# shahruk10/kaldi-tflite

Measured on AMD Instinct MI355X. Metric: x-vectors/sec (10 s @16 kHz), higher is better.
Workload: dtype f16mx

## Files before the change

### include/ktf_hip.h

```cpp
#ifndef KTF_HIP_H_
#define KTF_HIP_H_

#include <stddef.h>
#include <stdint.h>

#ifdef __cplusplus
extern "C" {
#endif

#define KTF_OK 0
#define KTF_EINVAL (-1)
#define KTF_ELAUNCH (-2)
#define KTF_EUNSUPPORTED (-3)

#define KTF_F32 0
#define KTF_BF16 1
#define KTF_BF16P 3

#define KTF_GEMM_F32 0
#define KTF_GEMM_BF16 1
#define KTF_GEMM_BF16X3 2
#define KTF_GEMM_F16MX 5
#define KTF_GEMM_BF16X4 6

// ... 51 lines not shown
    int32_t mel_stride;
    int32_t reserved;
} KtfFrontendTables;

#define KTF_IN_WAV 0
#define KTF_IN_FRAMES 1
#define KTF_IN_WINDOWED 2
#define KTF_IN_WAV_I16 3
#define KTF_OUT_FRAMES 0
#define KTF_OUT_WINDOWED 1
#define KTF_OUT_FBANK 2
#define KTF_OUT_MFCC 3

int64_t ktf_num_frames(int64_t n_samples, int32_t frame_size, int32_t frame_shift);
int64_t ktf_num_frames_padded(int64_t n_samples, int32_t frame_size, int32_t frame_shift, int32_t pad_mode);

int ktf_frontend_f32(const void* in, int64_t B, int64_t n, int32_t in_kind, const KtfFrontendCfg* cfg,
                     const KtfFrontendTables* tab, int32_t out_stage, float* out, float* energy,
                     uint64_t seed, void* stream);

int ktf_dct_f32(const float* x, int64_t rows, int32_t in_dim, int32_t out_dim, const float* dct,
                const float* lifter, float* out, void* stream);

typedef struct KtfVadCfg {
    float energy_threshold;
    float energy_mean_scale;
    float proportion_threshold;
    int32_t frames_context;
    int32_t energy_coeff;
} KtfVadCfg;

typedef struct KtfCmvnCfg {
    int32_t window;
    int32_t norm_vars;
    int32_t valid;
    int32_t reserved;
} KtfCmvnCfg;

int ktf_vad_mask_f32(const float* feats, int64_t B, int64_t T, int32_t D, const KtfVadCfg* cfg, float* mask,
                     void* stream);
int ktf_vad_index(const float* feats, int64_t B, int64_t T, int32_t D, const KtfVadCfg* cfg, int32_t* idx,
                  int32_t* lens, void* stream);
int ktf_cmvn_f32(const float* x, int64_t B, int64_t T, int32_t D, int64_t ldx, const int32_t* lens,
                 const KtfCmvnCfg* cfg, float* out, int64_t ldo, int32_t* out_lens, float* work, void* stream);
int ktf_vad_cmvn(const float* feats, int64_t B, int64_t T, int32_t D, const KtfVadCfg* vad, const KtfCmvnCfg* cmvn,
                 void* out, int32_t out_dtype, int64_t ldo, int32_t* lens, int32_t* idx_work, float* work,
                 void* stream);

typedef struct KtfVcPlan {
    int64_t pos_ints;
    int64_t stage_floats;
    int64_t bs_floats;
    int64_t col_floats;
    int64_t lds_bytes;
    int32_t nsplit;
    int32_t lds_form;
} KtfVcPlan;
int ktf_vad_cmvn_plan(int64_t B, int64_t T, int32_t D, int64_t ldo, KtfVcPlan* plan);
int ktf_cmvn_plan(int64_t T, int32_t D, int64_t ldo, KtfVcPlan* plan);

int ktf_route_short(const int32_t* lens, int64_t B, int32_t min_frames, int32_t* lens_main, int32_t* lens_short, int32_t* host_flag,
                    int32_t seq, void* stream);

typedef struct KtfTdnnDesc {
    int32_t units;
    int32_t din;
    int32_t din_pad;
    int32_t nctx;
    int32_t ctx[16];
    int32_t subsampling;
    int32_t valid;
    int32_t act;
    int32_t gemm;
    int32_t x_dtype, w_dtype, y_dtype;
    int32_t flags;
} KtfTdnnDesc;

#define KTF_TDNN_REF_TILES 1
#define KTF_TDNN_DET_STATS 2
#define KTF_TDNN_K_INTERLEAVED 4
#define KTF_TDNN_W_TILED 8

#define KTF_TDNN_MX_LOADER (1 << 24)

const char* ktf_tdnn_last_kernel(void);


int64_t ktf_tdnn_out_len(int64_t len, const KtfTdnnDesc* d);
int ktf_tdnn_out_lens(const int32_t* lens, int64_t B, const KtfTdnnDesc* d, int32_t* out_lens, void* stream);

int ktf_tdnn(const void* x, int64_t B, int64_t T, int64_t ldx, const int32_t* lens, const KtfTdnnDesc* d,
             const void* w, const void* w_lo, const float* bias, const float* scale, const float* shift,
             void* y, int64_t ldy, int32_t* out_lens, void* stream);

int ktf_tdnn_stats(const void* x, int64_t B, int64_t T, int64_t ldx, const int32_t* lens, const KtfTdnnDesc* d,
                   const void* w, const void* w_lo, const float* bias, const float* scale, const float* shift, double* sums,
                   void* stream);
int ktf_tdnn_split(const void* x_hi, const void* x_lo, int64_t B, int64_t T, int64_t ldx, const int32_t* lens,
                   const KtfTdnnDesc* d, const void* w, const void* w_lo, const float* bias, const float* scale,
                   const float* shift, void* y, void* y_lo, int64_t ldy, int32_t* out_lens, void* stream);
int ktf_tdnn_split_flat(const void* x_hi, const void* x_lo, int64_t B, int64_t T, int64_t ldx, const int32_t* row_starts, const int32_t* row_map,
                        const KtfTdnnDesc* d, const void* w, const void* w_lo, const float* bias, const float* scale,
                        const float* shift, void* y, void* y_lo, int64_t ldy, void* stream);
int64_t ktf_flat_stats_slots(int64_t T);
int64_t ktf_flat_row_map_rows(int64_t B, int64_t T);
int ktf_flat_row_map(const int32_t* row_starts, int64_t B, int64_t T, int32_t* map, void* stream);
int ktf_tdnn_split_flat_stats(const void* x_hi, const void* x_lo, int64_t B, int64_t T, int64_t ldx, const int32_t* row_starts,
                              const int32_t* row_map, const KtfTdnnDesc* d, const void* w, const void* w_lo, const float* bias, const float* scale,
                              const float* shift, double* sums, void* stream);
int ktf_stats_finalize_flat(const double* sums, int64_t slots, const int32_t* row_starts, int64_t T, int64_t B, int32_t D,
                            int32_t include_std, float eps, float* out, int64_t ld_out, void* stream);
int ktf_tdnn_split_stats(const void* x_hi, const void* x_lo, int64_t B, int64_t T, int64_t ldx, const int32_t* lens,
                         const KtfTdnnDesc* d, const void* w, const void* w_lo, const float* bias, const float* scale,
                         const float* shift, double* sums, void* stream);
int ktf_split_bf16(const float* src, int64_t rows, int32_t D, int64_t ld_src, void* hi, void* lo, int64_t ld_dst,
                   void* stream);
int ktf_split_bf16_rows(const float* src, int64_t B, int64_t T, int32_t D, int64_t ld_src, const int32_t* lens, void* hi, void* lo,
                        int64_t ld_dst, void* stream);
int ktf_mx_planes(const float* src, int64_t B, int64_t T, int32_t D, int64_t ld_src, const int32_t* lens, void* xh, void* xl4,
                  void* x4, void* xs, void* stream);
int ktf_tdnn_mx(const void* xh, const void* xl4, const void* x4, const void* xs, int64_t B, int64_t T, const int32_t* lens,
                const KtfTdnnDesc* d, const void* wh, const void* wq, const float* bias, const float* scale, const float* shift,
                void* yh, void* yl4, void* y4, void* ys, float* yf, int64_t ldy, void* stream);
int ktf_tdnn_mx_flat(const void* xh, const void* xl4, const void* x4, const void* xs, int64_t B, int64_t T, const int32_t* row_starts,
                     const int32_t* row_map, const KtfTdnnDesc* d, const void* wh, const void* wq, const float* bias, const float* scale,
                     const float* shift, void* yh, void* yl4, void* y4, void* ys, void* stream);
int ktf_tdnn_mx_flat_stats(const void* xh, const void* xl4, const void* x4, const void* xs, int64_t B, int64_t T, const int32_t* row_starts,
                           const int32_t* row_map, const KtfTdnnDesc* d, const void* wh, const void* wq, const float* bias, const float* scale,
                           const float* shift, double* sums, void* stream);
int ktf_tdnn_mx_stats(const void* xh, const void* xl4, const void* x4, const void* xs, int64_t B, int64_t T, const int32_t* lens,
                      const KtfTdnnDesc* d, const void* wh, const void* wq, const float* bias, const float* scale,
                      const float* shift, double* sums, void* stream);
int ktf_stats_finalize(const double* sums, const int32_t* lens, int64_t T, int64_t B, int32_t D, int32_t include_std,
                       float eps, float* out, int64_t ld_out, void* stream);
int64_t ktf_stats_slots(int64_t T);
int64_t ktf_tdnn_stats_slots(int64_t T, int32_t gemm);
int32_t ktf_tdnn_slot_rows(int32_t gemm);
int64_t ktf_mx_stats_slots(int64_t T, int32_t flags);
int32_t ktf_mx_slot_rows(int32_t flags);
int ktf_stats_finalize_slots(const double* sums, int64_t slots, int32_t slot_rows, const int32_t* lens, int64_t T, int64_t B, int32_t D,
                             int32_t include_std, float eps, float* out, int64_t ld_out, void* stream);

int ktf_activation_f32(float* y, int64_t B, int64_t T, int32_t D, int64_t ld, const int32_t* lens, int32_t act, const float* scale,
                       const float* shift, void* stream);

int ktf_affine_act_f32(const float* x, int64_t rows, int32_t D, int32_t act, const float* scale, const float* shift,
                       float* y, void* stream);
int ktf_convert_pad(const void* src, int32_t src_dtype, int64_t rows, int32_t D, int64_t ld_src, void* dst,
                    int32_t dst_dtype, int64_t ld_dst, void* stream);

int ktf_stats_pool(const void* x, int32_t x_dtype, int64_t B, int64_t T, int32_t D, int64_t ldx,
                   const int32_t* lens, int32_t input_period, int32_t include_std, float eps, float* out,
                   int64_t ld_out, void* stream);
int ktf_stats_pool_windowed_f32(const float* x, int64_t B, int64_t T, int32_t D, int32_t left, int32_t right,
                                int32_t input_period, int32_t output_period, int32_t start, int64_t T_out,
                                int32_t include_std, float eps, float* out, void* stream);

int ktf_xvec_tail_f32(const float* pooled, int64_t ld_pooled, const double* sums, int64_t slots, int32_t slot_rows, const int32_t* lens, int64_t T,
                      int64_t B, int32_t D, int32_t include_std, float eps, const float* W, int64_t ldw, const float* bias,
                      int32_t units, const float* mean, const float* A, const float* off, int32_t out_dim, float* partial,
                      uint32_t* counters, float* y, float* h_out, int32_t group, int32_t flags, void* stream);
#define KTF_TAIL_SKIP_EMPTY 1
int ktf_xvec_post_f32(const float* x, int64_t B, int32_t in_dim, int32_t out_dim, const float* mean, const float* A,
                      const float* off, float* y, void* stream);

int ktf_plda_f64(const double* x, int64_t B, int32_t dim, const double* A, const double* offset, const double* psi,
// ... 180 lines not shown
```

### kaldi-tflite_amd/csrc/tdnn_mx.hip

```cpp
#include "tdnn_mx_common.h"

#define MXP_ROWS 256
__global__ __launch_bounds__(MXP_ROWS) void mx_planes_kernel(const float* __restrict__ src, int64_t T, int64_t ld, int D,
                                                             const int32_t* __restrict__ lens, char* __restrict__ xh,
                                                             char* __restrict__ xl4, char* __restrict__ x4, char* __restrict__ xs) {
    __shared__ float tile[MXP_ROWS * 33];
    const int b = blockIdx.z, c = blockIdx.y, nch = gridDim.y;
    const int64_t t0 = (int64_t)blockIdx.x * MXP_ROWS;
    const int64_t len = lens ? (int64_t)lens[b] : T;
    if (t0 >= len) return;
    const int rows = (int)(len - t0 < MXP_ROWS ? len - t0 : MXP_ROWS);
    const int tid = threadIdx.x;
    const float* base = src + ((int64_t)b * T + t0) * ld + c * 32;
    const bool vec = (ld & 3) == 0 && ((uintptr_t)src & 15) == 0 && c * 32 + 32 <= ld;
#pragma unroll
    for (int k = 0; k < 8; ++k) {
        const int q = k * MXP_ROWS + tid, r = q >> 3, e4 = (q & 7) * 4;
        if (r < rows) {
            float v[4];
            if (vec) {
                const f32x4 t = *reinterpret_cast<const f32x4*>(base + (int64_t)r * ld + e4);
                const int nd = D - (c * 32 + e4);
                v[0] = nd > 0 ? t.x : 0.0f; v[1] = nd > 1 ? t.y : 0.0f; v[2] = nd > 2 ? t.z : 0.0f; v[3] = nd > 3 ? t.w : 0.0f;
            } else {
// ... 127 lines not shown
        }
        s_row = er[2].y;
        s_lm1 = er[2].z - 1;
        s_ub = er[2].x < 0 ? 0u : (unsigned)(er[2].x - er[2].y) * (unsigned)p.nch_in;
    }
    const unsigned vw = (unsigned)tid * 16u;
    const int wave_k0 = (int)(unsigned)(size_t)(lds_ptr_t*)(rsm + wave * 1024);
    [[maybe_unused]] const int wave_k = wave_k0;
#define MX_LDS_AT(off_, c_) ((lds_ptr_t*)(size_t)(unsigned)((off_) + (c_)))
    int kb[5], ko[5];
    kb[0] = MX_KQ_BIAS;
    ko[0] = MX_CTX(0);
#define MX_DMA_A_E(ks_, e_, n_)                                                                                        \
    {                                                                                                                  \
        int r_ = a_row[n_] + ko[e_];                                                                                   \
        const int hi_ = FLAT ? a_lm1[n_] : lenm1;                                                                      \
        r_ = r_ < 0 ? 0 : (r_ > hi_ ? hi_ : r_);                                                                       \
        const unsigned vo_ = ((FLAT ? a_ub[n_] : 0u) + (unsigned)r_) * 64u + a_cb[n_];                                 \
        __builtin_amdgcn_raw_ptr_buffer_load_lds(r_xh, MX_LDS_AT(wave_k, ((ks_) & 1) * MX_STAGE + (n_) * 8192), 16, vo_, kb[e_] << 6, 0, 0); \
    }
#define MX_DMA_A_I(ks_, e_, n_)                                                                                        \
    __builtin_amdgcn_raw_ptr_buffer_load_lds(r_xh, MX_LDS_AT(wave_k, ((ks_) & 1) * MX_STAGE + (n_) * 8192), 16, (n_) ? va1 : va0, \
                                             (kb[e_] + ko[e_]) << 6, 0, 0);
#define MX_DMA_A(ks_, e_, n_) { if constexpr (INTERIOR) MX_DMA_A_I(ks_, e_, n_) else MX_DMA_A_E(ks_, e_, n_) }
#define MX_DMA_W(ks_, n_)                                                                                              \
    __builtin_amdgcn_raw_ptr_buffer_load_lds(r_wh, MX_LDS_AT(wave_k, ((ks_) & 1) * MX_STAGE + MX_TILE + (n_) * 8192), 16, vw, \
                                             (ks_) * MX_TILE + (n_) * 8192, 0, 0);
    MX_DMA_W(0, 0) MX_DMA_W(0, 1) MX_DMA_A_E(0, 0, 0) MX_DMA_A_E(0, 0, 1)
    const __amdgpu_buffer_rsrc_t r_xl4 = mx_rsrc_pinned(p.xl4 + (ub - MX_KQ_BIAS) * 16);
    const __amdgpu_buffer_rsrc_t r_x4 = mx_rsrc_pinned(p.x4 + (ub - MX_KQ_BIAS) * 16);
    const __amdgpu_buffer_rsrc_t r_xs = mx_rsrc_pinned(p.xs + (ub - MX_KQ_BIAS) * 4);
    if constexpr (FLAT) {
        if (p.nctx == 1 && MX_CTX(0) == 0) {
            interior = true;
        } else if (out_len == 256) {
            const i32x4 e0 = flat_row(0), e1 = flat_row(255);
            interior = __builtin_amdgcn_readfirstlane(e0.w) == __builtin_amdgcn_readfirstlane(e1.w) &&
                       __builtin_amdgcn_readfirstlane(e0.y) + MX_CTX(0) >= 0 &&
                       __builtin_amdgcn_readfirstlane(e1.y) + MX_CTX(p.nctx - 1) <= __builtin_amdgcn_readfirstlane(e1.z) - 1;
        }
    }
    [[maybe_unused]] const unsigned va0 = (a_ub[0] + (unsigned)a_row[0]) * 64u + a_cb[0], va1 = (a_ub[1] + (unsigned)a_row[1]) * 64u + a_cb[1];
    [[maybe_unused]] const unsigned vs16 = (s_ub + (unsigned)s_row) * 16u, vs4 = (s_ub + (unsigned)s_row) * 4u;

    const int sa_k0 = (int)(unsigned)(size_t)(lds_ptr_t*)(rsm + (wave & 3) * 1024 + (wave >> 2) * 4096);
    const int sa_ks0 = (int)(unsigned)(size_t)(lds_ptr_t*)(rsm + (wave & 3) * 256 + (wave >> 2) * 1024);
    const bool wave_hi = wave >= 4;

    int* const tkb = reinterpret_cast<int*>(rsm + MX_KQ_OFF);
    int* const tko = tkb + (nkp + 4);

#define MX_DMA_SA(n_)                                                                                                  \
    {                                                                                                                  \
        constexpr int plane_ = ((n_) < 4 ? (n_) : 0) >> 1, h_ = (n_) < 4 ? ((n_) & 1) : (n_) - 4;                      \
        unsigned rec_ = 0u;                                                                                            \
        int so_;                                                                                                       \
        if constexpr (INTERIOR) {                                                                                      \
            so_ = sk_b[h_] + sk_o[h_];                                                                                 \
        } else {                                                                                                       \
            int r_ = s_row + sk_o[h_];                                                                                 \
            const int hi_ = FLAT ? s_lm1 : lenm1;                                                                      \
            r_ = r_ < 0 ? 0 : (r_ > hi_ ? hi_ : r_);                                                                   \
            rec_ = (FLAT ? s_ub : 0u) + (unsigned)r_;                                                                  \
            so_ = sk_b[h_];                                                                                            \
        }                                                                                                              \
        if ((n_) < 4) {                                                                                                \
            __builtin_amdgcn_raw_ptr_buffer_load_lds(plane_ ? r_x4 : r_xl4, MX_LDS_AT(sa_k, MX_SA_OFF + plane_ * 16384 + h_ * 8192), 16, \
                                                     INTERIOR ? vs16 : rec_ * 16u, so_ << 4, 0, 0);                    \
        } else {                                                                                                       \
            __builtin_amdgcn_raw_ptr_buffer_load_lds(r_xs, MX_LDS_AT(sa_ks, MX_SA_OFF + 32768 + h_ * 2048), 4, INTERIOR ? vs4 : rec_ * 4u, so_ << 2, 0, 0); \
        }                                                                                                              \
    }
#define MX_DMA_SW(ss_, n_)                                                                                             \
    __builtin_amdgcn_raw_ptr_buffer_load_lds(r_wq, MX_LDS_AT(wave_k, MX_SW_OFF + (n_) * 8192), 16, vw, (ss_) * MX_WQ_BLOCK + (n_) * 8192, 0, 0);

    f32x4 acc[8][4];
    const int r16 = lane & 15, q4 = lane >> 4;
    const int fr = (4 - ((r16 >> 2) & 3)) & 3;
    const int coff = ((q4 ^ fr) << 4);
    const int a_row_off = (wm * 128 + r16) * 64 + coff;
    const int b_row_off = (wn * 64 + r16) * 64 + coff;
    const int klim = PADK ? p.nk : nkp;

    auto kloop = [&](auto itag) {
        constexpr bool INTERIOR = decltype(itag)::value;
        {
            unsigned char* const prm_w = rsm + MX_PRM_OFF + (wave & 3) * 256;
            const unsigned vcol = (unsigned)(n0 + (wave & 3) * 64 + lane) * 4u;
            const float* const vec0 = wave_hi ? p.scale : p.bias;
            if (vec0) __builtin_amdgcn_raw_ptr_buffer_load_lds(mx_rsrc(vec0, p.units * 4), (lds_ptr_t*)(prm_w + (wave_hi ? 1024 : 0)), 4, vcol, 0, 0, 0);
            else reinterpret_cast<float*>(prm_w + (wave_hi ? 1024 : 0))[lane] = wave_hi ? 1.0f : 0.0f;
            if (!wave_hi) {
                if (p.shift) __builtin_amdgcn_raw_ptr_buffer_load_lds(mx_rsrc(p.shift, p.units * 4), (lds_ptr_t*)(prm_w + 2048), 4, vcol, 0, 0, 0);
                else reinterpret_cast<float*>(prm_w + 2048)[lane] = 0.0f;
            }
        }
        for (int k = tid; k < nkp + 4; k += 512) {
            const int kk = k + 1 < p.nk ? k + 1 : 0;
            const int ch = kk / p.nctx, ci = kk - ch * p.nctx;
            tkb[k] = ch * (int)p.T + MX_KQ_BIAS;
            tko[k] = MX_CTX(ci);
        }
        {
            int ch = 0, ci = 0;
#pragma unroll
            for (int e = 1; e <= 4; ++e) {
                if (++ci == p.nctx) { ci = 0; ++ch; }
                const bool real = e < p.nk;
                kb[e] = (real ? ch * (int)p.T : 0) + MX_KQ_BIAS;
                ko[e] = real ? MX_CTX(ci) : MX_CTX(0);
            }
        }
#pragma unroll
        for (int i = 0; i < 8; ++i)
#pragma unroll
            for (int j = 0; j < 4; ++j) acc[i][j] = f32x4{0.0f, 0.0f, 0.0f, 0.0f};
        for (int ss = 0; ss < p.nss; ++ss) {
            i32x4 tb_n, to_n;
            int sk_b[2], sk_o[2];
            int wave_k = wave_k0, sa_k = sa_k0, sa_ks = sa_ks0;
            asm volatile("" : "+s"(wave_k), "+s"(sa_k), "+s"(sa_ks));
#pragma unroll
            for (int j = 0; j < 4; ++j) {
                const int ks = 4 * ss + j;
                if (j == 1 || j == 2) asm volatile("s_waitcnt vmcnt(6)" ::: "memory");
                else if (j == 0) asm volatile("s_waitcnt vmcnt(0) lgkmcnt(0)" ::: "memory");
                else asm volatile("s_waitcnt vmcnt(0)" ::: "memory");
                __builtin_amdgcn_s_barrier();
                asm volatile("" ::: "memory");
                const bool live = PADK ? ks < p.nk : true;
#define MX_NEXT() ({ int k1_ = ks + 1; asm volatile("" : "+s"(k1_)); k1_ < klim; })
                const unsigned char* sa = rsm + (ks & 1) * MX_STAGE;
                const unsigned char* sw = sa + MX_TILE;
                hfrag8 bh[4];
                hfrag8 a_cur, a_nx1;
                if (live) {
#pragma unroll
                    for (int jj = 0; jj < 4; ++jj) bh[jj] = *reinterpret_cast<const hfrag8*>(sw + b_row_off + jj * 1024);
                    a_cur = *reinterpret_cast<const hfrag8*>(sa + a_row_off);
                    a_nx1 = *reinterpret_cast<const hfrag8*>(sa + a_row_off + 1024);
                }
                __builtin_amdgcn_sched_barrier(0);
                if (MX_NEXT()) { MX_DMA_A(ks + 1, j + 1, 0) MX_DMA_A(ks + 1, j + 1, 1) }
                __builtin_amdgcn_sched_barrier(0);
#pragma unroll
                for (int i = 0; i < 8; ++i) {
                    if (live) {
                        acc[i][0] = __builtin_amdgcn_mfma_f32_16x16x32_f16(a_cur, bh[0], acc[i][0], 0, 0, 0);
                        __builtin_amdgcn_sched_barrier(0);
                        hfrag8 a_nx2 = a_nx1;
                        if (i < 6) a_nx2 = *reinterpret_cast<const hfrag8*>(sa + a_row_off + (i + 2) * 1024);
#pragma unroll
                        for (int jj = 1; jj < 4; ++jj) acc[i][jj] = __builtin_amdgcn_mfma_f32_16x16x32_f16(a_cur, bh[jj], acc[i][jj], 0, 0, 0);
                        a_cur = a_nx1;
                        a_nx1 = a_nx2;
                    }
                    __builtin_amdgcn_sched_barrier(0);
                    if (i == 0) { if (MX_NEXT()) MX_DMA_W(ks + 1, 0) }
                    if (i == 1) { if (MX_NEXT()) MX_DMA_W(ks + 1, 1) }
                    if (j == 0) {
                        if (i == 1) {
                            sk_b[0] = wave_hi ? kb[1] : kb[0]; sk_o[0] = wave_hi ? ko[1] : ko[0];
                            sk_b[1] = wave_hi ? kb[3] : kb[2]; sk_o[1] = wave_hi ? ko[3] : ko[2];
                        }
                        if (i == 2) MX_DMA_SA(0)
                        if (i == 3) MX_DMA_SA(1)
                        if (i == 4) MX_DMA_SA(2)
                        if (i == 5) MX_DMA_SA(3)
                        if (i == 6) MX_DMA_SA(4)
                        if (i == 7) MX_DMA_SA(5)
                    }
                    if (j == 1) {
                        if (i == 2) MX_DMA_SW(ss, 0)
                        if (i == 3) MX_DMA_SW(ss, 1)
                        if (i == 4) MX_DMA_SW(ss, 2)
                        if (i == 5) MX_DMA_SW(ss, 3)
                        if (i == 6) MX_DMA_SW(ss, 4)
                        if (i == 7) MX_DMA_SW(ss, 5)
                    }
                    if (j == 2 && i == 3) {
                        tb_n = *reinterpret_cast<const i32x4*>(tkb + 4 * ss + 4);
                        to_n = *reinterpret_cast<const i32x4*>(tko + 4 * ss + 4);
                    }
                    __builtin_amdgcn_sched_barrier(0);
                }
#undef MX_NEXT
            }
            __builtin_amdgcn_sched_barrier(0);
            {
                int tl;
                asm volatile("v_mbcnt_lo_u32_b32 %0, -1, 0\n\tv_mbcnt_hi_u32_b32 %0, -1, %0" : "=v"(tl));
                const int sw_rec = ((tl & 63) >> 4) * 256 + wn * 64 + (tl & 15);
                const int sa_rec = ((tl & 63) >> 4) * 256 + wm * 128 + (tl & 15);
                unsigned o_a16 = MX_SA_OFF + sa_rec * 16, o_a4 = MX_SA_OFF + 32768 + sa_rec * 4;
                asm volatile("" : "+v"(o_a16), "+v"(o_a4));
                const unsigned char* const pa16 = rsm + o_a16;
                const unsigned char* const pa4 = rsm + o_a4;
                unsigned o_w16 = MX_SW_OFF + sw_rec * 16, o_w8 = MX_SW_OFF + 32768 + sw_rec * 8, o_w4 = MX_SW_OFF + 40960 + sw_rec * 4;
                asm volatile("" : "+v"(o_w16), "+v"(o_w8), "+v"(o_w4));
                const unsigned char* const pw16 = rsm + o_w16;
                const unsigned char* const pw8 = rsm + o_w8;
                const unsigned char* const pw4 = rsm + o_w4;
                u32x4 w4[4], wl6a[4];
                u32x2 wl6b[4];
                unsigned wsc[4];
#pragma unroll
                for (int jj = 0; jj < 4; ++jj) {
                    w4[jj] = *reinterpret_cast<const u32x4*>(pw16 + jj * 256);
                    wl6a[jj] = *reinterpret_cast<const u32x4*>(pw16 + 16384 + jj * 256);
                    wl6b[jj] = *reinterpret_cast<const u32x2*>(pw8 + jj * 128);
                    wsc[jj] = *reinterpret_cast<const unsigned*>(pw4 + jj * 64);
                }
                u32x4 l_n = *reinterpret_cast<const u32x4*>(pa16);
                u32x4 h_n = *reinterpret_cast<const u32x4*>(pa16 + 16384);
                unsigned s_n = *reinterpret_cast<const unsigned*>(pa4);
#pragma unroll
                for (int i = 0; i < 8; ++i) {
                    const u32x4 l = l_n, h = h_n;
                    const unsigned asc = s_n;
                    if (i < 7) {
                        l_n = *reinterpret_cast<const u32x4*>(pa16 + (i + 1) * 256);
                        h_n = *reinterpret_cast<const u32x4*>(pa16 + 16384 + (i + 1) * 256);
                        s_n = *reinterpret_cast<const unsigned*>(pa4 + (i + 1) * 64);
                    }
                    const i32x8 al = i32x8{(int)l.x, (int)l.y, (int)l.z, (int)l.w, 0, 0, 0, 0};
                    const i32x8 ah = i32x8{(int)h.x, (int)h.y, (int)h.z, (int)h.w, 0, 0, 0, 0};
#pragma unroll
                    for (int jj = 0; jj < 4; ++jj) {
                        const i32x8 bw = i32x8{(int)w4[jj].x, (int)w4[jj].y, (int)w4[jj].z, (int)w4[jj].w, 0, 0, 0, 0};
                        acc[i][jj] = __builtin_amdgcn_mfma_scale_f32_16x16x128_f8f6f4(al, bw, acc[i][jj], 4, 4, 0, asc, 0, wsc[jj]);
                    }
#pragma unroll
                    for (int jj = 0; jj < 4; ++jj) {
                        const i32x8 bw = i32x8{(int)wl6a[jj].x, (int)wl6a[jj].y, (int)wl6a[jj].z, (int)wl6a[jj].w, (int)wl6b[jj].x, (int)wl6b[jj].y, 0, 0};
                        acc[i][jj] = __builtin_amdgcn_mfma_scale_f32_16x16x128_f8f6f4(ah, bw, acc[i][jj], 4, 2, 1, asc, 1, wsc[jj]);
                    }
                    if (i == 3) {
                        kb[0] = kb[4];
                        ko[0] = ko[4];
#pragma unroll
                        for (int e = 0; e < 4; ++e) {
                            kb[e + 1] = __builtin_amdgcn_readfirstlane(tb_n[e]);
                            ko[e + 1] = __builtin_amdgcn_readfirstlane(to_n[e]);
                        }
                    }
                    __builtin_amdgcn_sched_barrier(0);
                }
            }
        }
    };
    if constexpr (FLAT) {
        if (interior) kloop(std::true_type{});
        else kloop(std::false_type{});
    } else {
        kloop(std::false_type{});
    }
#undef MX_DMA_A
#undef MX_DMA_A_E
#undef MX_DMA_A_I
#undef MX_DMA_W
#undef MX_DMA_SA
#undef MX_DMA_SW
#undef MX_ARG_BATCH
#undef MX_LDS_AT
#undef MX_CTX

#include "tdnn_mx_epilogue.inc"
}

template <int ACT, int OUT, bool PADK, bool FLAT = false>
__global__ __launch_bounds__(512) void tdnn_mx_kernel(MxParams p, int mtiles, int ntiles, int gtiles, double* __restrict__ stats) {
    extern __shared__ __attribute__((aligned(16))) unsigned char rsm[];
    mx_tile<ACT, OUT, PADK, FLAT>(p, blockIdx.x, mtiles, ntiles, gtiles, stats, rsm);
}

static int mx_launch(const void* xh, const void* xl4, const void* x4, const void* xs, int64_t B, int64_t T, const int32_t* lens,
                     const KtfTdnnDesc* d, const void* wh, const void* wq, const float* bias, const float* scale, const float* shift,
                     void* yh, void* yl4, void* y4, void* ys, float* yf, int64_t ldy, double* stats, void* stream, const char* who,
                     const int32_t* row_starts = nullptr, const int32_t* row_map = nullptr) {
    KTF_REQUIRE(d && wh && wq, "%s: null argument", who);
    KTF_REQUIRE(d->gemm == KTF_GEMM_F16MX, "%s: needs KTF_GEMM_F16MX", who);
    KTF_REQUIRE(B >= 0 && T >= 0 && B < 65536, "%s: bad size", who);
    KTF_REQUIRE(B == 0 || T == 0 || (xh && xl4 && x4 && xs), "%s: null argument", who);
    if (const int rc = tdnn_check_desc(d, scale, shift, who); rc != KTF_OK) return rc;
    KTF_REQUIRE(d->subsampling <= 64, "%s: subsampling %d outside [1,64]", who, d->subsampling);
    const bool plain = !d->valid && d->subsampling == 1;
    KTF_REQUIRE(plain || !stats, "%s: the fused pooling takes SAME padding without subsampling", who);
    KTF_REQUIRE(d->act == KTF_ACT_NONE || d->act == KTF_ACT_RELU, "%s: fuses ReLU or no activation", who);
    KTF_REQUIRE(T * (int64_t)d->din_pad * 2 < (1ll << 31) - (1ll << 20), "%s: T * din_pad too large", who);
    KTF_REQUIRE((((int64_t)d->din_pad / 32 * d->nctx + 3) / 4) * 4 <= MX_KQ_MAX_STEPS || (d->flags & KTF_TDNN_MX_LOADER), "%s: more than %d K-steps (din_pad / 32 * contexts)", who, MX_KQ_MAX_STEPS);
    if (B == 0 || T == 0 || ktf_tdnn_out_len(T, d) <= 0) return KTF_OK;
    const int outs = (yh ? 1 : 0) + (yf ? 1 : 0) + (stats ? 1 : 0);
    KTF_REQUIRE(outs == 1, "%s: exactly one of the plane / fp32 / pooled outputs", who);
    if (yh) KTF_REQUIRE(yl4 && y4 && ys, "%s: a plane output needs all four planes", who);
    if (yf) KTF_REQUIRE(ldy >= d->units, "%s: ldy < units", who);
    if (B == 0 || T == 0) return KTF_OK;
    MxParams p;
    memset(&p, 0, sizeof(p));
    p.xh = (const char*)xh; p.xl4 = (const char*)xl4; p.x4 = (const char*)x4; p.xs = (const char*)xs;
    p.lens = lens; p.wh = (const char*)wh; p.wq = (const char*)wq; p.bias = bias; p.scale = scale; p.shift = shift;
    p.yh = (char*)yh; p.yl4 = (char*)yl4; p.y4 = (char*)y4; p.ys = (char*)ys; p.yf = yf; p.ldy = ldy; p.T = T;
    p.units = d->units; p.nch_in = d->din_pad / 32; p.nctx = d->nctx; p.nk = p.nch_in * d->nctx; p.nss = (p.nk + 3) / 4;
    p.nch_out = (d->units + 31) / 32;
    p.sub = d->subsampling;
    p.start = (d->valid && d->ctx[0] < 0) ? -d->ctx[0] : 0;
    p.cut = (d->valid && d->ctx[d->nctx - 1] > 0) ? d->ctx[d->nctx - 1] : 0;
    p.Tout = ktf_tdnn_out_len(T, d);
    if (p.Tout <= 0) return KTF_OK;
    KTF_REQUIRE(plain || !(d->flags & KTF_TDNN_MX_LOADER), "%s: the loader-wave kernel takes SAME padding without subsampling", who);
    const bool loader = (d->flags & KTF_TDNN_MX_LOADER) != 0;
    p.stat_slots = (stats && (d->flags & KTF_TDNN_DET_STATS)) ? (int32_t)ktf_mx_stats_slots(T, d->flags) : 0;
    for (int i = 0; i < d->nctx; ++i) {
        KTF_REQUIRE(d->ctx[i] >= -128 && d->ctx[i] <= 127, "%s: context offsets outside [-128, 127]", who);
        p.ctx_pk[i >> 3] |= (unsigned long long)(unsigned char)(signed char)d->ctx[i] << ((i & 7) * 8);
    }
    hipStream_t st = (hipStream_t)stream;
    const int o = stats ? MX_OUT_STATS : (yf ? MX_OUT_F32 : MX_OUT_PLANES);
    if (loader) {
        const int rc = mxl_launch(p, B, d->act, o, stats, st);
        if (rc != KTF_OK) return rc;
        KTF_CHECK_LAUNCH(who);
        return KTF_OK;
    }
    if (row_starts) {
        KTF_REQUIRE(row_map && plain && o != MX_OUT_F32 && !loader, "%s: flat row tiles take the row table, SAME padding, no subsampling, a plane or pooled output", who);
        p.stat_slots = (stats && (d->flags & KTF_TDNN_DET_STATS)) ? (int32_t)ktf_flat_stats_slots(T) : 0;
        KTF_REQUIRE(B <= 4095 && B * T * (int64_t)p.nch_in * 64 < (1ll << 32) - (1ll << 20) && B * T < (1ll << 31) / (p.nch_out > 0 ? p.nch_out : 1),
                    "%s: flat row tiles need B <= 4095 and B * T * din_pad * 2 < 2^32", who);
        p.row_starts = row_starts; p.row_map = row_map;
        if (T > 1) {
            uint32_t l = 0;
            while ((1ull << l) < (uint64_t)T) ++l;
            p.t_div_m = (uint32_t)((1ull << (31 + l)) / (uint64_t)T + 1);
            p.t_div_s = l - 1;
        }
        const int ntiles = ktf_cdiv(d->units, 256);
        const int64_t ftiles = ktf_cdiv(B * T, 256);
        const int64_t fblocks = grouped_blocks(ftiles, ntiles);
        tdnn_pick<MX_OUT_STATS, MX_OUT_PLANES>(o, [&](auto O) {
            tdnn_pick<KTF_ACT_RELU, KTF_ACT_NONE>(d->act, [&](auto A) {
                tdnn_pick<true, false>((p.nk & 3) != 0, [&](auto PADK) {
                    tdnn_launch_kernel<tdnn_mx_kernel<A, O, PADK, true>>("tdnn_mx_kernel<flat>", dim3((unsigned)fblocks), dim3(512), MX_LDS_TOTAL(p.nss * 4),
                                                                         MX_LDS_TOTAL(MX_KQ_MAX_STEPS), st, p, (int)B, ntiles, (int)ftiles, stats);
                });
            });
        });
        KTF_CHECK_LAUNCH(who);
        return KTF_OK;
    }
    const int mtiles = ktf_cdiv(p.Tout, 256), ntiles = ktf_cdiv(d->units, 256);
    const int64_t gtiles = B * mtiles;
    const int64_t nblocks = grouped_blocks(gtiles, ntiles);
    tdnn_pick<KTF_ACT_RELU, KTF_ACT_NONE>(d->act, [&](auto A) {
        tdnn_pick<MX_OUT_STATS, MX_OUT_F32, MX_OUT_PLANES>(o, [&](auto O) {
            tdnn_pick<true, false>((p.nk & 3) != 0, [&](auto PADK) {
                tdnn_launch_kernel<tdnn_mx_kernel<A, O, PADK>>("tdnn_mx_kernel", dim3((unsigned)nblocks), dim3(512), MX_LDS_TOTAL(p.nss * 4),
                                                               MX_LDS_TOTAL(MX_KQ_MAX_STEPS), st, p, mtiles, ntiles, (int)gtiles, stats);
            });
        });
    });
    KTF_CHECK_LAUNCH(who);
    return KTF_OK;
}

extern "C" int ktf_tdnn_mx(const void* xh, const void* xl4, const void* x4, const void* xs, int64_t B, int64_t T, const int32_t* lens,
                           const KtfTdnnDesc* d, const void* wh, const void* wq, const float* bias, const float* scale,
                           const float* shift, void* yh, void* yl4, void* y4, void* ys, float* yf, int64_t ldy, void* stream) {
    return mx_launch(xh, xl4, x4, xs, B, T, lens, d, wh, wq, bias, scale, shift, yh, yl4, y4, ys, yf, ldy, nullptr, stream, "ktf_tdnn_mx");
}

extern "C" int ktf_tdnn_mx_flat(const void* xh, const void* xl4, const void* x4, const void* xs, int64_t B, int64_t T, const int32_t* row_starts,
                                const int32_t* row_map, const KtfTdnnDesc* d, const void* wh, const void* wq, const float* bias, const float* scale,
                                const float* shift, void* yh, void* yl4, void* y4, void* ys, void* stream) {
    KTF_REQUIRE(B == 0 || T == 0 || (row_starts && row_map && yh), "ktf_tdnn_mx_flat: null argument");
    return mx_launch(xh, xl4, x4, xs, B, T, nullptr, d, wh, wq, bias, scale, shift, yh, yl4, y4, ys, nullptr, 0, nullptr, stream, "ktf_tdnn_mx_flat",
                     row_starts, row_map);
}

extern "C" int ktf_tdnn_mx_flat_stats(const void* xh, const void* xl4, const void* x4, const void* xs, int64_t B, int64_t T, const int32_t* row_starts,
                                      const int32_t* row_map, const KtfTdnnDesc* d, const void* wh, const void* wq, const float* bias,
                                      const float* scale, const float* shift, double* sums, void* stream) {
    KTF_REQUIRE(sums && (B == 0 || T == 0 || (row_starts && row_map)), "ktf_tdnn_mx_flat_stats: null argument");
    return mx_launch(xh, xl4, x4, xs, B, T, nullptr, d, wh, wq, bias, scale, shift, nullptr, nullptr, nullptr, nullptr, nullptr, 0, sums, stream,
                     "ktf_tdnn_mx_flat_stats", row_starts, row_map);
}

extern "C" int ktf_tdnn_mx_stats(const void* xh, const void* xl4, const void* x4, const void* xs, int64_t B, int64_t T,
                                 const int32_t* lens, const KtfTdnnDesc* d, const void* wh, const void* wq, const float* bias,
                                 const float* scale, const float* shift, double* sums, void* stream) {
    KTF_REQUIRE(sums, "ktf_tdnn_mx_stats: null sums");
    return mx_launch(xh, xl4, x4, xs, B, T, lens, d, wh, wq, bias, scale, shift, nullptr, nullptr, nullptr, nullptr, nullptr, 0, sums, stream,
                     "ktf_tdnn_mx_stats");
}

extern "C" int32_t ktf_mx_slot_rows(int32_t flags) { return (flags & KTF_TDNN_MX_LOADER) ? 96 : 128; }
extern "C" int64_t ktf_mx_stats_slots(int64_t T, int32_t flags) {
    if (!(flags & KTF_TDNN_MX_LOADER)) return ktf_stats_slots(T);
    return T <= 0 ? 2 : 2 * ((T + 191) / 192);
}
```

### kaldi-tflite_amd/csrc/tdnn_mx_common.h

```cpp
#pragma once
#include "tdnn_common.h"
#include "flat_stats.h"
#include <type_traits>

typedef __attribute__((ext_vector_type(8))) int i32x8;
typedef __attribute__((ext_vector_type(8))) _Float16 hfrag8;
typedef __attribute__((ext_vector_type(2))) unsigned u32x2;

#define MX_TILE 16384
#define MX_STAGE (2 * MX_TILE)
#define MX_SA_OFF (2 * MX_STAGE)
#define MX_SA_BYTES (2 * 16384 + 4096)
#define MX_SW_OFF (MX_SA_OFF + MX_SA_BYTES)
#define MX_WQ_BLOCK 49152
#define MX_PRM_OFF (MX_SW_OFF + MX_WQ_BLOCK)
#define MX_LDS_BYTES (MX_PRM_OFF + 3 * 256 * 4)
#define MX_KQ_OFF MX_LDS_BYTES
#define MX_KQ_BIAS 128
#define MX_KQ_MAX_STEPS 1144
#define MX_LDS_TOTAL(nkp) (MX_LDS_BYTES + 8 * ((nkp) + 4))
static_assert(8 * 64 * 68 * 4 <= MX_PRM_OFF, "epilogue staging regions");
#define MX_EPW_PITCH 68

struct MxParams {
    const char* xh;
    const char* xl4;
    const char* x4;
    const char* xs;
    const int32_t* lens;
    const char* wh;
    const char* wq;
    const float* bias;
    const float* scale;
    const float* shift;
    char* yh;
    char* yl4;
    char* y4;
    char* ys;
    float* yf;
    int64_t ldy;
    int64_t T;
    int64_t Tout;
    int32_t units, nch_in, nctx, nk, nss, nch_out, stat_slots;
    int32_t sub, start, cut;
    unsigned long long ctx_pk[2];
    const int32_t* row_starts;
    const int32_t* row_map;
    uint32_t t_div_m, t_div_s;
};

__device__ __forceinline__ __amdgpu_buffer_rsrc_t mx_rsrc(const void* ptr, int bytes = -1) {
    return __builtin_amdgcn_make_buffer_rsrc(const_cast<void*>(ptr), 0, bytes, 0x00020000);
}
typedef int mx_rs4 __attribute__((ext_vector_type(4)));
__device__ __forceinline__ __amdgpu_buffer_rsrc_t mx_rsrc_pinned(const void* ptr, int bytes = -1) {
    const unsigned long long a = (unsigned long long)ptr;
    mx_rs4 w{(int)(unsigned)a, (int)((unsigned)(a >> 32) & 0xffffu), bytes, 0x00020000};
    asm volatile("" : "+s"(w));
    __amdgpu_buffer_rsrc_t r;
    __builtin_memcpy(&r, &w, 16);
    return r;
}

__device__ __forceinline__ unsigned mx_fp4_scale_byte(float m) {
    const unsigned bits = __float_as_uint(m);
    int byte = (int)(bits >> 23) - 2 + ((bits & 0x7fffffu) >= 0x600000u ? 1 : 0);
    return (unsigned)(byte < 1 ? 1 : byte);
}


__device__ __forceinline__ int mx_unit(int cb, int m) { return (cb >> 1) * 32 + (m >> 2) * 8 + (cb & 1) * 4 + (m & 3); }

__device__ __forceinline__ void mx_transpose4(unsigned& a, unsigned& b, unsigned& c, unsigned& d) {
    auto r = __builtin_amdgcn_permlane16_swap(a, b, false, false); a = r[0]; b = r[1];
    r = __builtin_amdgcn_permlane16_swap(c, d, false, false); c = r[0]; d = r[1];
    r = __builtin_amdgcn_permlane32_swap(a, c, false, false); a = r[0]; c = r[1];
    r = __builtin_amdgcn_permlane32_swap(b, d, false, false); b = r[0]; d = r[1];
}

template <int N>
__device__ __forceinline__ void mx_encode8(const float (&v)[N][8], u32x4 (&hp)[N], unsigned (&l4)[N], unsigned (&h4)[N], unsigned (&sw)[N]) {
    typedef __attribute__((ext_vector_type(2))) float f2;
    typedef __attribute__((ext_vector_type(2))) _Float16 h2;
    float lo[N][8];
    unsigned hw[N][4];
    float mv[N], ml[N];
#pragma unroll
    for (int n = 0; n < N; ++n) { mv[n] = 0.0f; ml[n] = 0.0f; }
#pragma unroll
    for (int k = 0; k < 4; ++k) {
#pragma unroll
        for (int n = 0; n < N; ++n) {
            const float a = v[n][2 * k], b = v[n][2 * k + 1];
            const h2 hh = __builtin_convertvector(f2{a, b}, h2);
            hw[n][k] = __builtin_bit_cast(unsigned, hh);
            asm("v_fma_mix_f32 %0, -%1, 1.0, %2 op_sel_hi:[1,0,0]" : "=v"(lo[n][2 * k]) : "v"(hw[n][k]), "v"(a));
            asm("v_fma_mix_f32 %0, -%1, 1.0, %2 op_sel:[1,0,0] op_sel_hi:[1,0,0]" : "=v"(lo[n][2 * k + 1]) : "v"(hw[n][k]), "v"(b));
            asm("v_max3_f32 %0, |%1|, |%2|, %3" : "=v"(mv[n]) : "v"(a), "v"(b), "v"(mv[n]));
            asm("v_max3_f32 %0, |%1|, |%2|, %3" : "=v"(ml[n]) : "v"(lo[n][2 * k]), "v"(lo[n][2 * k + 1]), "v"(ml[n]));
        }
    }
#pragma unroll
    for (int step = 0; step < 2; ++step) {
        unsigned o[N][2][2];
#pragma unroll
        for (int n = 0; n < N; ++n) {
            if (step == 0) {
                auto r = __builtin_amdgcn_permlane16_swap(__float_as_uint(mv[n]), __float_as_uint(mv[n]), false, false);
                o[n][0][0] = r[0]; o[n][0][1] = r[1];
                r = __builtin_amdgcn_permlane16_swap(__float_as_uint(ml[n]), __float_as_uint(ml[n]), false, false);
                o[n][1][0] = r[0]; o[n][1][1] = r[1];
            } else {
                auto r = __builtin_amdgcn_permlane32_swap(__float_as_uint(mv[n]), __float_as_uint(mv[n]), false, false);
                o[n][0][0] = r[0]; o[n][0][1] = r[1];
                r = __builtin_amdgcn_permlane32_swap(__float_as_uint(ml[n]), __float_as_uint(ml[n]), false, false);
                o[n][1][0] = r[0]; o[n][1][1] = r[1];
            }
        }
#pragma unroll
        for (int n = 0; n < N; ++n) {
            asm("v_max_f32 %0, %1, %2" : "=v"(mv[n]) : "v"(o[n][0][0]), "v"(o[n][0][1]));
            asm("v_max_f32 %0, %1, %2" : "=v"(ml[n]) : "v"(o[n][1][0]), "v"(o[n][1][1]));
        }
    }
    float sh[N], sl[N];
#pragma unroll
    for (int n = 0; n < N; ++n) {
        const float mh = (float)(_Float16)mv[n];
        const unsigned bh = mx_fp4_scale_byte(mh), bl = mx_fp4_scale_byte(ml[n]);
        sh[n] = __uint_as_float(bh << 23);
        sl[n] = __uint_as_float(bl << 23);
// ... 83 lines not shown
```

Measured before the change: 110,800.

## Add specialized single-channel first-layer MX kernel path with preloaded weights

Adds a dedicated k-loop variant for the first TDNN layer (one input channel, five context taps, small context span). It preloads the whole input tile including the halo and all weight tiles into a custom LDS map in one batch of DMAs. It then runs unrolled f16 MFMA steps with staged vmcnt waits, followed by scaled-MX steps, and skips the generic per-step ring pipeline and k-table indexing. The cost is a larger LDS footprint for this path, which may lower occupancy, and a lot of hand-scheduled code; an opt-out flag selects the old ring path.

```diff
diff --git a/include/ktf_hip.h b/include/ktf_hip.h
--- a/include/ktf_hip.h
+++ b/include/ktf_hip.h
@@ -157,6 +157,7 @@
 #define KTF_TDNN_W_TILED 8
 
 #define KTF_TDNN_MX_LOADER (1 << 24)
+#define KTF_TDNN_MX_RING (1 << 25)
 
 const char* ktf_tdnn_last_kernel(void);
 
diff --git a/kaldi-tflite_amd/csrc/tdnn_mx.hip b/kaldi-tflite_amd/csrc/tdnn_mx.hip
--- a/kaldi-tflite_amd/csrc/tdnn_mx.hip
+++ b/kaldi-tflite_amd/csrc/tdnn_mx.hip
@@ -233,19 +233,21 @@
     const int b_row_off = (wn * 64 + r16) * 64 + coff;
     const int klim = PADK ? p.nk : nkp;
 
+    auto prm_dma = [&]() {
+        unsigned char* const prm_w = rsm + MX_PRM_OFF + (wave & 3) * 256;
+        const unsigned vcol = (unsigned)(n0 + (wave & 3) * 64 + lane) * 4u;
+        const float* const vec0 = wave_hi ? p.scale : p.bias;
+        if (vec0) __builtin_amdgcn_raw_ptr_buffer_load_lds(mx_rsrc(vec0, p.units * 4), (lds_ptr_t*)(prm_w + (wave_hi ? 1024 : 0)), 4, vcol, 0, 0, 0);
+        else reinterpret_cast<float*>(prm_w + (wave_hi ? 1024 : 0))[lane] = wave_hi ? 1.0f : 0.0f;
+        if (!wave_hi) {
+            if (p.shift) __builtin_amdgcn_raw_ptr_buffer_load_lds(mx_rsrc(p.shift, p.units * 4), (lds_ptr_t*)(prm_w + 2048), 4, vcol, 0, 0, 0);
+            else reinterpret_cast<float*>(prm_w + 2048)[lane] = 0.0f;
+        }
+    };
+
     auto kloop = [&](auto itag) {
         constexpr bool INTERIOR = decltype(itag)::value;
-        {
-            unsigned char* const prm_w = rsm + MX_PRM_OFF + (wave & 3) * 256;
-            const unsigned vcol = (unsigned)(n0 + (wave & 3) * 64 + lane) * 4u;
-            const float* const vec0 = wave_hi ? p.scale : p.bias;
-            if (vec0) __builtin_amdgcn_raw_ptr_buffer_load_lds(mx_rsrc(vec0, p.units * 4), (lds_ptr_t*)(prm_w + (wave_hi ? 1024 : 0)), 4, vcol, 0, 0, 0);
-            else reinterpret_cast<float*>(prm_w + (wave_hi ? 1024 : 0))[lane] = wave_hi ? 1.0f : 0.0f;
-            if (!wave_hi) {
-                if (p.shift) __builtin_amdgcn_raw_ptr_buffer_load_lds(mx_rsrc(p.shift, p.units * 4), (lds_ptr_t*)(prm_w + 2048), 4, vcol, 0, 0, 0);
-                else reinterpret_cast<float*>(prm_w + 2048)[lane] = 0.0f;
-            }
-        }
+        prm_dma();
         for (int k = tid; k < nkp + 4; k += 512) {
             const int kk = k + 1 < p.nk ? k + 1 : 0;
             const int ch = kk / p.nctx, ci = kk - ch * p.nctx;
@@ -400,8 +402,170 @@
             }
         }
     };
+    [[maybe_unused]] auto kfirst = [&](auto nkt) {
+        constexpr int NK = decltype(nkt)::value;
+        const int c_min = MX_CTX(0), span = MX_CTX(p.nctx - 1) - c_min;
+        constexpr bool two = NK > 4;
+        int wave_k = wave_k0;
+        int lds0 = (int)(unsigned)(size_t)(lds_ptr_t*)rsm;
+        asm volatile("" : "+s"(wave_k), "+s"(lds0));
+        const int w4 = wave & 3;
+        prm_dma();
+        const int so_a = MX_KQ_BIAS + c_min;
+        if (!wave_hi) __builtin_amdgcn_raw_ptr_buffer_load_lds(r_xl4, MX_LDS_AT(lds0, MX_F1_XL4_OFF + w4 * 1024), 16, vs16, so_a << 4, 0, 0);
+        else __builtin_amdgcn_raw_ptr_buffer_load_lds(r_x4, MX_LDS_AT(lds0, MX_F1_X4_OFF + w4 * 1024), 16, vs16, so_a << 4, 0, 0);
+        {
+            const int last = 255 + span;
+            const unsigned d_a = (unsigned)(min(256 + (lane >> 2), last) - (tid >> 2));
+            const unsigned d_s = (unsigned)(min(256 + lane, last) - (lane + 64 * w4));
+            if (!wave_hi) __builtin_amdgcn_raw_ptr_buffer_load_lds(r_xs, MX_LDS_AT(lds0, MX_F1_XS_OFF + w4 * 256), 4, vs4, so_a << 2, 0, 0);
+            else if (wave == 4) __builtin_amdgcn_raw_ptr_buffer_load_lds(r_xh, MX_LDS_AT(lds0, MX_F1_HALO_OFF), 16, va0 + d_a * 64u, so_a << 6, 0, 0);
+            else if (wave == 5) __builtin_amdgcn_raw_ptr_buffer_load_lds(r_xl4, MX_LDS_AT(lds0, MX_F1_XL4_OFF + 4096), 16, vs16 + d_s * 16u, so_a << 4, 0, 0);
+            else if (wave == 6) __builtin_amdgcn_raw_ptr_buffer_load_lds(r_x4, MX_LDS_AT(lds0, MX_F1_X4_OFF + 4096), 16, vs16 + d_s * 16u, so_a << 4, 0, 0);
+            else __builtin_amdgcn_raw_ptr_buffer_load_lds(r_xs, MX_LDS_AT(lds0, MX_F1_XS_OFF + 1024), 4, vs4 + d_s * 4u, so_a << 2, 0, 0);
+        }
+#define MX_F1_DMA_W(k_, so_, n_) \
+    __builtin_amdgcn_raw_ptr_buffer_load_lds(r_wh, MX_LDS_AT(wave_k, MX_F1_W_OFF(k_) + (n_) * 8192), 16, vw, (so_) + (n_) * 8192, 0, 0);
+#define MX_F1_DMA_SW(dst_, ss_, n_) \
+    __builtin_amdgcn_raw_ptr_buffer_load_lds(r_wq, MX_LDS_AT(wave_k, (dst_) + (n_) * 8192), 16, vw, (ss_) * MX_WQ_BLOCK + (n_) * 8192, 0, 0);
+        MX_F1_DMA_W(1, 1 * MX_TILE, 0) MX_F1_DMA_W(1, 1 * MX_TILE, 1) MX_F1_DMA_W(2, 2 * MX_TILE, 0) MX_F1_DMA_W(2, 2 * MX_TILE, 1)
+        MX_F1_DMA_W(3, 3 * MX_TILE, 0) MX_F1_DMA_W(3, 3 * MX_TILE, 1)
+        MX_F1_DMA_SW(MX_F1_SW_OFF, 0, 0) MX_F1_DMA_SW(MX_F1_SW_OFF, 0, 1) MX_F1_DMA_SW(MX_F1_SW_OFF, 0, 2) MX_F1_DMA_SW(MX_F1_SW_OFF, 0, 3)
+        MX_F1_DMA_SW(MX_F1_SW_OFF, 0, 4)
+        if (!wave_hi) MX_F1_DMA_SW(MX_F1_SW_OFF, 0, 5)
+        {
+            const int so4 = two ? 4 * MX_TILE : 0;
+            MX_F1_DMA_W(4, so4, 0) MX_F1_DMA_W(4, so4, 1)
+        }
+#pragma unroll
+        for (int i = 0; i < 8; ++i)
+#pragma unroll
+            for (int j = 0; j < 4; ++j) acc[i][j] = f32x4{0.0f, 0.0f, 0.0f, 0.0f};
+        int f_ab, f_a7;
+#define MX_F1_FRAG(ab_, a7_, off_)                                                                                     \
+        {                                                                                                              \
+            int tl_;                                      \
+            asm volatile("v_mbcnt_lo_u32_b32 %0, -1, 0\n\tv_mbcnt_hi_u32_b32 %0, -1, %0" : "=v"(tl_));               \
+            const int R_ = (tl_ & 15) + (off_);                                                                        \
+            ab_ = (wm * 128 + R_) * 64 + (((tl_ >> 4) ^ ((0 - (R_ >> 2)) & 3)) << 4);                                  \
+            a7_ = ab_ + 7 * 1024 + ((wm == 1 && R_ >= 16) ? MX_F1_HALO_OFF - MX_TILE : 0);                             \
+        }
+        MX_F1_FRAG(f_ab, f_a7, 0)
+        auto fstep = [&](auto kt, auto vt, auto dt) {
+            constexpr int k = decltype(kt)::value, vm = decltype(vt)::value;
+            constexpr bool SIDE_W1 = decltype(dt)::value;
+            if constexpr (k == 0) asm volatile("s_waitcnt vmcnt(%0) lgkmcnt(0)" ::"n"(vm) : "memory");
+            else asm volatile("s_waitcnt vmcnt(%0)" ::"n"(vm) : "memory");
+            __builtin_amdgcn_s_barrier(); asm volatile("" ::: "memory");
+            if constexpr (k < NK) {
+                const unsigned char* sw = rsm + MX_F1_W_OFF(k);
+                hfrag8 bh[4];
+#pragma unroll
+                for (int jj = 0; jj < 4; ++jj) bh[jj] = *reinterpret_cast<const hfrag8*>(sw + b_row_off + jj * 1024);
+                hfrag8 a_cur = *reinterpret_cast<const hfrag8*>(rsm + f_ab);
+                hfrag8 a_nx1 = *reinterpret_cast<const hfrag8*>(rsm + f_ab + 1024);
+                __builtin_amdgcn_sched_barrier(0);
+#pragma unroll
+                for (int i = 0; i < 8; ++i) {
+                    acc[i][0] = __builtin_amdgcn_mfma_f32_16x16x32_f16(a_cur, bh[0], acc[i][0], 0, 0, 0);
+                    __builtin_amdgcn_sched_barrier(0);
+                    hfrag8 a_nx2 = a_nx1;
+                    if (i < 5) a_nx2 = *reinterpret_cast<const hfrag8*>(rsm + f_ab + (i + 2) * 1024);
+                    else if (i == 5) a_nx2 = *reinterpret_cast<const hfrag8*>(rsm + f_a7);
+#pragma unroll
+                    for (int jj = 1; jj < 4; ++jj) acc[i][jj] = __builtin_amdgcn_mfma_f32_16x16x32_f16(a_cur, bh[jj], acc[i][jj], 0, 0, 0);
+                    a_cur = a_nx1;
+                    a_nx1 = a_nx2;
+                    __builtin_amdgcn_sched_barrier(0);
+                    if constexpr (SIDE_W1) {
+                        if (i >= 2) MX_F1_DMA_SW(MX_F1_W_OFF(0), 1, i - 2)
+                    }
+                    if constexpr (k < 4) {
+                        if (i == 6) MX_F1_FRAG(f_ab, f_a7, k + 1 < NK ? MX_CTX(k + 1) - c_min : 0)
+                    }
+                    __builtin_amdgcn_sched_barrier(0);
+                }
+            }
+        };
+        auto mstep = [&](auto st) {
+            constexpr int ss = decltype(st)::value;
+            constexpr int swb = ss == 0 ? MX_F1_SW_OFF : MX_F1_W_OFF(0);
+            __builtin_amdgcn_sched_barrier(0);
+            int tl;
+            asm volatile("v_mbcnt_lo_u32_b32 %0, -1, 0\n\tv_mbcnt_hi_u32_b32 %0, -1, %0" : "=v"(tl));
+            const int kblk = 4 * ss + ((tl & 63) >> 4);
+            const int koff = kblk < NK ? (int)(signed char)(cpk0 >> (kblk * 8)) - c_min : 0;
+            const int sw_rec = ((tl & 63) >> 4) * 256 + wn * 64 + (tl & 15);
+            const int sa_rec = wm * 128 + (tl & 15) + koff;
+            unsigned o_al = MX_F1_XL4_OFF + sa_rec * 16, o_ah = MX_F1_X4_OFF + sa_rec * 16, o_a4 = MX_F1_XS_OFF + sa_rec * 4;
+            asm volatile("" : "+v"(o_al), "+v"(o_ah), "+v"(o_a4));
+            const unsigned char* const pal = rsm + o_al;
+            const unsigned char* const pah = rsm + o_ah;
+            const unsigned char* const pa4 = rsm + o_a4;
+            unsigned o_w16 = swb + sw_rec * 16, o_w8 = swb + 32768 + sw_rec * 8, o_w4 = swb + 40960 + sw_rec * 4;
+            asm volatile("" : "+v"(o_w16), "+v"(o_w8), "+v"(o_w4));
+            const unsigned char* const pw16 = rsm + o_w16;
+            const unsigned char* const pw8 = rsm + o_w8;
+            const unsigned char* const pw4 = rsm + o_w4;
+            u32x4 w4r[4], wl6a[4];
+            u32x2 wl6b[4];
+            unsigned wsc[4];
+#pragma unroll
+            for (int jj = 0; jj < 4; ++jj) {
+                w4r[jj] = *reinterpret_cast<const u32x4*>(pw16 + jj * 256);
+                wl6a[jj] = *reinterpret_cast<const u32x4*>(pw16 + 16384 + jj * 256);
+                wl6b[jj] = *reinterpret_cast<const u32x2*>(pw8 + jj * 128);
+                wsc[jj] = *reinterpret_cast<const unsigned*>(pw4 + jj * 64);
+            }
+            u32x4 l_n = *reinterpret_cast<const u32x4*>(pal);
+            u32x4 h_n = *reinterpret_cast<const u32x4*>(pah);
+            unsigned s_n = *reinterpret_cast<const unsigned*>(pa4);
+#pragma unroll
+            for (int i = 0; i < 8; ++i) {
+                const u32x4 l = l_n, h = h_n;
+                const unsigned asc = s_n;
+                if (i < 7) {
+                    l_n = *reinterpret_cast<const u32x4*>(pal + (i + 1) * 256);
+                    h_n = *reinterpret_cast<const u32x4*>(pah + (i + 1) * 256);
+                    s_n = *reinterpret_cast<const unsigned*>(pa4 + (i + 1) * 64);
+                }
+                const i32x8 al = i32x8{(int)l.x, (int)l.y, (int)l.z, (int)l.w, 0, 0, 0, 0};
+                const i32x8 ah = i32x8{(int)h.x, (int)h.y, (int)h.z, (int)h.w, 0, 0, 0, 0};
+#pragma unroll
+                for (int jj = 0; jj < 4; ++jj) {
+                    const i32x8 bw = i32x8{(int)w4r[jj].x, (int)w4r[jj].y, (int)w4r[jj].z, (int)w4r[jj].w, 0, 0, 0, 0};
+                    acc[i][jj] = __builtin_amdgcn_mfma_scale_f32_16x16x128_f8f6f4(al, bw, acc[i][jj], 4, 4, 0, asc, 0, wsc[jj]);
+                }
+#pragma unroll
+                for (int jj = 0; jj < 4; ++jj) {
+                    const i32x8 bw = i32x8{(int)wl6a[jj].x, (int)wl6a[jj].y, (int)wl6a[jj].z, (int)wl6a[jj].w, (int)wl6b[jj].x, (int)wl6b[jj].y, 0, 0};
+                    acc[i][jj] = __builtin_amdgcn_mfma_scale_f32_16x16x128_f8f6f4(ah, bw, acc[i][jj], 4, 2, 1, asc, 1, wsc[jj]);
+                }
+                __builtin_amdgcn_sched_barrier(0);
+            }
+        };
+#define MX_F1_STEP(k_, vm_, d_) fstep(std::integral_constant<int, k_>{}, std::integral_constant<int, vm_>{}, std::integral_constant<bool, d_>{});
+        MX_F1_STEP(0, 13, false) MX_F1_STEP(1, 11, false) MX_F1_STEP(2, 9, false)
+        MX_F1_STEP(3, 2, two)
+        mstep(std::integral_constant<int, 0>{});
+        if constexpr (two) {
+            MX_F1_STEP(4, 6, false)
+            asm volatile("s_waitcnt vmcnt(0)" ::: "memory");
+            __builtin_amdgcn_s_barrier(); asm volatile("" ::: "memory");
+            mstep(std::integral_constant<int, 1>{});
+        }
+        asm volatile("s_waitcnt vmcnt(0)" ::: "memory");
+#undef MX_F1_STEP
+#undef MX_F1_FRAG
+#undef MX_F1_DMA_W
+#undef MX_F1_DMA_SW
+    };
     if constexpr (FLAT) {
-        if (interior) kloop(std::true_type{});
+        if constexpr (PADK && OUT == MX_OUT_PLANES) {
+            if (interior && p.first) kfirst(std::integral_constant<int, 5>{});
+            else if (interior) kloop(std::true_type{});
+            else kloop(std::false_type{});
+        } else if (interior) kloop(std::true_type{});
         else kloop(std::false_type{});
     } else {
         kloop(std::false_type{});
@@ -488,10 +652,16 @@
         const int ntiles = ktf_cdiv(d->units, 256);
         const int64_t ftiles = ktf_cdiv(B * T, 256);
         const int64_t fblocks = grouped_blocks(ftiles, ntiles);
+        int lds = MX_LDS_TOTAL(p.nss * 4);
+        if (o == MX_OUT_PLANES && p.nch_in == 1 && p.nk == 5 && d->ctx[d->nctx - 1] - d->ctx[0] <= MX_F1_MAX_SPAN &&
+            !(d->flags & KTF_TDNN_MX_RING)) {
+            p.first = 1;
+            lds = MX_F1_LDS_BYTES > lds ? MX_F1_LDS_BYTES : lds;
+        }
         tdnn_pick<MX_OUT_STATS, MX_OUT_PLANES>(o, [&](auto O) {
             tdnn_pick<KTF_ACT_RELU, KTF_ACT_NONE>(d->act, [&](auto A) {
                 tdnn_pick<true, false>((p.nk & 3) != 0, [&](auto PADK) {
-                    tdnn_launch_kernel<tdnn_mx_kernel<A, O, PADK, true>>("tdnn_mx_kernel<flat>", dim3((unsigned)fblocks), dim3(512), MX_LDS_TOTAL(p.nss * 4),
+                    tdnn_launch_kernel<tdnn_mx_kernel<A, O, PADK, true>>("tdnn_mx_kernel<flat>", dim3((unsigned)fblocks), dim3(512), lds,
                                                                          MX_LDS_TOTAL(MX_KQ_MAX_STEPS), st, p, (int)B, ntiles, (int)ftiles, stats);
                 });
             });
diff --git a/kaldi-tflite_amd/csrc/tdnn_mx_common.h b/kaldi-tflite_amd/csrc/tdnn_mx_common.h
--- a/kaldi-tflite_amd/csrc/tdnn_mx_common.h
+++ b/kaldi-tflite_amd/csrc/tdnn_mx_common.h
@@ -21,6 +21,15 @@
 #define MX_LDS_TOTAL(nkp) (MX_LDS_BYTES + 8 * ((nkp) + 4))
 static_assert(8 * 64 * 68 * 4 <= MX_PRM_OFF, "epilogue staging regions");
 #define MX_EPW_PITCH 68
+#define MX_F1_MAX_SPAN 16
+#define MX_F1_W_OFF(k) (MX_TILE * ((k) + 1))
+#define MX_F1_SW_OFF MX_F1_W_OFF(5)
+#define MX_F1_X4_OFF (MX_F1_SW_OFF + MX_WQ_BLOCK - 4096)
+#define MX_F1_HALO_OFF (MX_F1_X4_OFF + 320 * 16)
+#define MX_F1_XS_OFF (MX_F1_HALO_OFF + 1024)
+#define MX_F1_XL4_OFF MX_LDS_TOTAL(8)
+#define MX_F1_LDS_BYTES (MX_F1_XL4_OFF + 320 * 16)
+static_assert(MX_F1_XS_OFF + 320 * 4 <= MX_PRM_OFF && MX_F1_LDS_BYTES <= MX_LDS_TOTAL(MX_KQ_MAX_STEPS), "first-layer form: LDS map");
 
 struct MxParams {
     const char* xh;
@@ -47,6 +56,7 @@
     const int32_t* row_starts;
     const int32_t* row_map;
     uint32_t t_div_m, t_div_s;
+    int32_t first;
 };
 
 __device__ __forceinline__ __amdgpu_buffer_rsrc_t mx_rsrc(const void* ptr, int bytes = -1) {
```

After: 111,300, median of 4. No clear change (+0.4%).
